# mhostetter/gr-adsb

Measured on AMD Instinct MI355X. Metric: IQ Msamples/s through framer+demod, higher is better.
Workload: dtype f32

## Files before the change

gr_adsb_amd/csrc/adsb_device.h:

```cpp
#pragma once

#ifndef ADSB_ROUTE
#define ADSB_ROUTE(id, offset) ((void)0)
#endif
#ifndef ADSB_AIR_MIN
#if defined(__HIP__)
#define ADSB_AIR_MIN(p, v) __hip_atomic_fetch_min((p), (v), __ATOMIC_RELAXED, __HIP_MEMORY_SCOPE_AGENT)
#define ADSB_AIR_LOAD(p) __hip_atomic_load((p), __ATOMIC_RELAXED, __HIP_MEMORY_SCOPE_AGENT)
#define ADSB_AIR_STORE(p, v) __hip_atomic_store((p), (v), __ATOMIC_RELAXED, __HIP_MEMORY_SCOPE_AGENT)
#else
#define ADSB_AIR_MIN(p, v) atomicMin((p), (v))
#define ADSB_AIR_LOAD(p) (*(p))
#define ADSB_AIR_STORE(p, v) ((void)(*(p) = (v)))
#endif
#endif
#ifndef ADSB_COLD_AT
#define ADSB_COLD_AT(e) (e)
#endif

namespace adsb {

enum Route : int {
  kRouteWindow = 0,
  kRoutePend = 1,
  kRoutePendFull = 2,
  kRouteFlush = 3,
  kRouteLongFast = 4,
  kRouteLongClipped = 5,
  kRouteCount = 6
};

constexpr int kThreads = 256;
constexpr int kWaves = kThreads / 64;
constexpr int kWTile = 1024;
constexpr int kFwd = 256;
constexpr int kBack = 128;
constexpr int kWWin = kWTile + kFwd;
constexpr int kMaxCentre = (kWTile - 1 + kWWin - 1) / 2;
template <bool B> struct BoolC { static constexpr bool value = B; };
constexpr int kWWords = kWWin / 64;
constexpr int kWOwn = kWTile / 64;
constexpr int kHeadWords = kFwd / 64;
constexpr unsigned kTemplate = 0x285u;
constexpr int kNoise = 100;
constexpr long long kNoIndex = -(1ll << 62);
static_assert(kWOwn == 16 && kFwd % 64 == 0, "word owners are lanes 0..15 of each wavefront");
static_assert(kBack % 64 == 0 && kBack >= 100, "the noise window of a centre in the tile must lie in the LDS window");

constexpr int kMinWaves = 5;

enum RecFlags : unsigned {
  kDemod = 1u,
  kKept = 2u,
  kNoMatch = 4u,
  kPending = 8u,
  kHead = 16u,
  kLongHint = 32u,
  kParityOk = 32u,
  kLongFmt = 64u,
  kKnownDf = 128u,
  kDfShift = 8u,
  kRecLongHint = 0x2000u,
  kFecFixed = 0x4000u,
  kFecDf = 0x8000u,
  kApFec = 4u,
  kApKnown = 8u,
};

struct CrcTab { unsigned r[112]; };
constexpr CrcTab make_crc_tab() {
  CrcTab t{};
  unsigned v = 1;
  for (int j = 0; j < 112; ++j) {
    t.r[j] = v;
    v <<= 1;
    if (v & 0x1000000u) v ^= 0x1FFF409u;
  }
  return t;
}
constexpr unsigned kDfShortSet = (1u << 0) | (1u << 4) | (1u << 5) | (1u << 11);
constexpr unsigned kDfLongSet = (1u << 16) | (1u << 17) | (1u << 18) | (1u << 19) | (1u << 20) | (1u << 21) | (1u << 24);
constexpr unsigned kDfPiSet = (1u << 11) | (1u << 17) | (1u << 18) | (1u << 19);

struct alignas(16) Rec { unsigned long long w[4]; };
struct alignas(16) RecHalf { unsigned long long a, b; };

constexpr long long kBias = 1ll << 40;
__device__ __forceinline__ unsigned long long cand_make(long long p, unsigned flags) {
  return ((unsigned long long)flags << 56) | (unsigned long long)(p + kBias);
}
__device__ __forceinline__ long long cand_p(unsigned long long c) {
  return (long long)(c & 0x00FFFFFFFFFFFFFFull) - kBias;
}
__device__ __forceinline__ unsigned cand_flags(unsigned long long c) { return (unsigned)(c >> 56); }

struct LongRise { long long rise; int blk; int slot; };

struct Summary {
  int n_rec;
  int n_kept;
  int overflow;
  int long_count;
  unsigned flags;
  int pad_;
  long long lastp;
  long long last_kept_p;
};

struct DetectArgs {
  const void* data;
  long long n;
  long long in0_base;
  long long scan_lo;
  long long scan_hi;
  long long fall_hi;
  long long dem_hi;
  long long origin;
  long long chunk;
  float thr;
  float prev_in0;
  float scale;
  int sps;
  int end_is_call_end;
  int long_aware;
  int rec_cap;
  int long_cap;
  unsigned long long* cands;
  Rec* recs;
  int* blk_count;
  long long* blk_lastp;
  unsigned* blk_flags;
  LongRise* longlist;
  int* long_count;
  unsigned long long* long_lastp;
};

__device__ __forceinline__ float mag2f(float re, float im) {
  return __fadd_rn(__fmul_rn(re, re), __fmul_rn(im, im));
}

__device__ __forceinline__ float mag2_iq16(unsigned iq, float scale) {
  const float re = __fmul_rn((float)(short)(iq & 0xFFFFu), scale);
  const float im = __fmul_rn((float)(short)(iq >> 16), scale);
  return mag2f(re, im);
}

constexpr int kModeSc8Pow2 = 5;
constexpr int kModeCu8Pow2 = 6;
template <int MODE>
__device__ __forceinline__ float mag2_iq8(unsigned iq, float scale) {
  if constexpr (MODE == 3 || MODE == kModeSc8Pow2) {
    const int i8 = (int)(signed char)(iq & 0xFFu), q8 = (int)(signed char)((iq >> 8) & 0xFFu);
    return mag2f(__fmul_rn((float)i8, scale), __fmul_rn((float)q8, scale));
  } else {
    const float fi = (float)(iq & 0xFFu), fq = (float)((iq >> 8) & 0xFFu);
    const float ci = __builtin_fmaf(fi, 2.0f, -255.0f), cq = __builtin_fmaf(fq, 2.0f, -255.0f);
    return mag2f(__fmul_rn(ci, scale), __fmul_rn(cq, scale));
  }
}

constexpr bool mode_is_iq8(int mode) { return mode == 3 || mode == 4 || mode == 5 || mode == 6; }
constexpr int det_waves(int mode) { return mode_is_iq8(mode) ? 1 : kWaves; }
constexpr int mode_bytes(int mode) { return mode == 0 ? 8 : mode_is_iq8(mode) ? 2 : 4; }

template <int MODE> struct RawSel { using type = float; };
template <> struct RawSel<0> { using type = float2; };
template <> struct RawSel<2> { using type = unsigned; };
template <> struct RawSel<3> { using type = unsigned short; };
template <> struct RawSel<4> { using type = unsigned short; };
template <> struct RawSel<5> { using type = unsigned short; };
template <> struct RawSel<6> { using type = unsigned short; };

template <int MODE>
__device__ __forceinline__ typename RawSel<MODE>::type load_raw(const void* data, long long i) {
  return reinterpret_cast<const typename RawSel<MODE>::type*>(data)[i];
}
template <int MODE>
__device__ __forceinline__ float raw_mag2(typename RawSel<MODE>::type r, float scale) {
  if constexpr (MODE == 0) return mag2f(r.x, r.y);
  else if constexpr (MODE == 2) return mag2_iq16(r, scale);
  else if constexpr (mode_is_iq8(MODE)) return mag2_iq8<MODE>(r, scale);
  else return r;
}

template <int MODE>
__device__ __forceinline__ float load_sample(const void* data, long long i, float scale) {
  return raw_mag2<MODE>(load_raw<MODE>(data, i), scale);
}

template <int MODE>
__device__ __forceinline__ float xg(const void* data, long long n, long long i, float scale) {
  if (i < 0 || i >= n) return 0.0f;
  return load_sample<MODE>(data, i, scale);
}

template <int MODE>
__device__ __forceinline__ float xg_nb(const void* data, long long n, long long i, float scale) {
  const bool ok = (i >= 0) & (i < n);
  const long long ci = ok ? i : 0;
  const float v = load_sample<MODE>(data, ci, scale);
  return ok ? v : 0.0f;
}

template <int MODE, class A>
__device__ __forceinline__ bool above_at(const A& a, long long i) {
  if (i >= 0) return xg<MODE>(a.data, a.n, i, a.scale) >= a.thr;
  if (i == a.in0_base - 1) return a.prev_in0 >= a.thr;
  return 0.0f >= a.thr;
}

__device__ __forceinline__ unsigned long long bit_range(long long lo, long long hi) {
  if (hi <= 0 || lo >= 64 || hi <= lo) return 0ull;
  if (lo < 0) lo = 0;
  if (hi > 64) hi = 64;
  unsigned long long m = (hi == 64) ? ~0ull : ((1ull << hi) - 1ull);
  return m & ~((1ull << lo) - 1ull);
}
// ... 903 lines not shown
        }
        adsb_wave_sync();

        const bool easy = it >= it_e0 && it < it_e1;
        if (easy) rises_to_records(BoolC<true>{}, it, t0, nr, lane);
        else rises_to_records(BoolC<false>{}, it, t0, nr, lane);
        adsb_setprio<0>();
      }
    }

    if (n_pend > 0 && it + 1 == ntile) {
      adsb_wave_sync();
      pend_flush<MODE, STAGED>(pend, n_pend, WinArgs<decltype(cold())>{cold(), a.origin, a.scale, a.sps}, s_x, t0, st, lane);
      n_pend = 0;
    }
    {
      const float4 keep = *reinterpret_cast<const float4*>(s_x + kWTile + 4 * lane);
      const float2 keepb = *reinterpret_cast<const float2*>(s_x + kWTile - kBack + 2 * lane);
      const unsigned short keepm = s_m16[kTileUnits + (lane & (kHeadUnits - 1))];
      adsb_wave_sync();
      *reinterpret_cast<float4*>(s_x + 4 * lane) = keep;
      *reinterpret_cast<float2*>(s_x - kBack + 2 * lane) = keepb;
      s_m16[lane & (kHeadUnits - 1)] = keepm;
    }
    pred = keepp;
    prev_active = active;
  };

  const int lane_outer = lane;
  if (cold()->n >= kWTile) {
    const char* const clamp = reinterpret_cast<const char*>(cold()->data) + (((cold()->n - kWTile) * (long long)BPS) & ~15ll);
    const char* nb = reinterpret_cast<const char*>(cold()->data) + (c0 + kFwd) * (long long)BPS;
    constexpr int D = (MODE == kModeSc8Pow2 || MODE == kModeCu8Pow2) ? 2 : 1;
    Body<MODE> body[D];
    if (ntile > 0) {
      body_issue(body[0], it_rag > 0 ? nb : clamp, lane);
#pragma unroll
      for (int d = 1; d < D; ++d) {
        nb += (long long)kWTile * BPS;
        body_issue(body[d], d - 1 < it_re ? nb : clamp, lane);
      }
      head_fill(lane);
    }
    auto step = [&](Body<MODE>& b, const int it, const bool real) {
      const int lane = adsb_opaque(lane_outer);
      const long long t0 = c0 + (long long)it * kWTile;
      nb += (long long)kWTile * BPS;
      constexpr bool MASKS = mode_is_iq8(MODE);
      unsigned bm_regs = 0u;
      bool active = false;
      const int mx = body_commit<MODE, true, MASKS>(b, s_x + kFwd, a.scale, lane, it + D - 1 < it_re ? nb : clamp, thr, thr_bits,
                                                    thr_pos, &bm_regs, &active);
      if (real) {
        if constexpr (!MASKS) active = !thr_pos || __ballot(mx >= thr_bits) != 0ull;
        if (it >= it_rag) {
          adsb_wave_sync();
          for (int i = lane; i < kWTile; i += 64) s_x[kFwd + i] = xg<MODE>(cold()->data, cold()->n, t0 + kFwd + i, a.scale);
          active = true;
        }
        process_tile(it, t0, active, lane, MASKS && it < it_rag, bm_regs);
      }
    };
    for (int it = 0; it < ntile; it += D) {
      step(body[0], it, true);
#pragma unroll
      for (int d = 1; d < D; ++d) step(body[d], it + d, it + d < ntile);
    }
  } else {
    if (ntile > 0) head_fill(lane_outer);
    for (int it = 0; it < ntile; ++it) {
      const int lane = adsb_opaque(lane_outer);
      const long long t0 = c0 + (long long)it * kWTile;
      for (int i = lane; i < kWTile; i += 64) s_x[kFwd + i] = xg<MODE>(cold()->data, cold()->n, t0 + kFwd + i, a.scale);
      process_tile(it, t0, true, lane, false, 0u);
    }
  }
  if (STAGED) stage_flush(st, nrec < a.rec_cap ? nrec : a.rec_cap, lane_outer);
#pragma unroll
  for (int d2 = 32; d2 >= 1; d2 >>= 1) lp = imax(lp, __shfl_xor(lp, d2));
  if (lane == 0) {
    cold()->blk_count[unit] = nrec;
    cold()->blk_lastp[unit] = lp >= 0 ? c0 + lp : kNoIndex;
    cold()->blk_flags[unit] = uflags;
  }
}
template <int MODE, int HALF>
__global__ void __launch_bounds__(64 * det_waves(MODE), kMinWaves) k_detect(DetectArgs a) {
  detect_body<MODE, HALF, det_waves(MODE)>(a, (int)blockIdx.x);
}

template <int MODE>
__device__ __forceinline__ void longrun_entry(const DetectArgs& a, int e) {
  __shared__ unsigned long long s_found;
  const int tid = threadIdx.x, lane = tid & 63, wave = tid >> 6;
  {
    const LongRise le = a.longlist[e];
    const long long limit = a.fall_hi;
    const long long start = le.rise + 1;
    const unsigned long long none = ~0ull;
    if (tid == 0) s_found = none;
    __syncthreads();
    for (long long base = start; base < limit; base += 4ll * kThreads) {
      unsigned long long mine = none;
      for (int q = 3; q >= 0; --q) {
        const long long i = base + 4ll * tid + q;
        if (i < limit && !above_at<MODE>(a, i)) mine = (unsigned long long)(i - start);
      }
      if (mine != none) atomicMin(&s_found, mine);
      __syncthreads();
      const bool done = s_found != none;
      __syncthreads();
      if (done) break;
    }
    __syncthreads();
    const long long f = (s_found == none) ? limit : start + (long long)s_found;
    unsigned long long* out = a.cands + (long long)le.blk * a.rec_cap + le.slot;
    if (wave == 0) {
      if (f < limit) {
        const long long p = (le.rise + f) >> 1;
        if (lane == 0) atomicMax(a.long_lastp, (unsigned long long)(p + (1ll << 62)));
        const float hp = __fmul_rn(xg<MODE>(a.data, a.n, p, a.scale), 0.5f);
        const float v = (lane < 16) ? xg<MODE>(a.data, a.n, p + (long long)lane * (a.sps >> 1), a.scale) : 0.0f;
        const unsigned long long cm = __ballot(lane < 16 && v > hp);
        unsigned hint = 0u;
        if (a.long_aware) {
          const long long i1 = p + 8ll * a.sps;
          if (xg<MODE>(a.data, a.n, i1, a.scale) > xg<MODE>(a.data, a.n, i1 + (a.sps >> 1), a.scale)) hint = kLongHint;
        }
        const bool match = (unsigned)cm == kTemplate;
        if (lane == 0) *out = match ? cand_make(p, hint) : cand_make(p, kNoMatch);
        if (match) {
          const BurstFetch<MODE> bf = burst_issue<MODE>(a, cand_make(p, hint), lane);
          burst_finish<MODE>(a, bf, a.recs + (long long)le.blk * a.rec_cap + le.slot, lane);
        }
      } else if (lane == 0) {
        *out = cand_make(le.rise, kNoMatch);
        if (!a.end_is_call_end) atomicOr(a.blk_flags + le.blk, 4u);
      }
    }
    __syncthreads();
  }
}
template <int MODE>
__device__ __forceinline__ void longrun_body(int bid, int nb, const DetectArgs& a) {
  int n_entries = *a.long_count;
  if (n_entries > a.long_cap) n_entries = a.long_cap;
  for (int e = bid; e < n_entries; e += nb) longrun_entry<MODE>(a, e);
}

__device__ __forceinline__ int block_excl_scan(int v, int* total) {
  __shared__ int s_wsum[kWaves];
  const int lane = threadIdx.x & 63, wave = threadIdx.x >> 6;
  int incl = v;
#pragma unroll
  for (int d = 1; d < 64; d <<= 1) {
    const int t = __shfl_up(incl, (unsigned)d);
    if (lane >= d) incl += t;
  }
  if (lane == 63) s_wsum[wave] = incl;
  __syncthreads();
  int base = 0, tot = 0;
#pragma unroll
  for (int w = 0; w < kWaves; ++w) {
    const int c = s_wsum[w];
    if (w < wave) base += c;
    tot += c;
// ... 2 lines not shown
  *total = tot;
  return base + incl - v;
}

constexpr int kScanRound = 512;
constexpr int kScanRoundBig = 2048;
template <int ROUND>
__device__ __forceinline__ void scan_body(const int* blk_count, const long long* blk_lastp,
                                          const unsigned* blk_flags, int nblk, int rec_cap,
                                          const int* long_count, const unsigned long long* long_lastp,
                                          int* blk_off, Summary* sum, int* s_cnt) {
  constexpr int kScanRound = ROUND;
  constexpr int kScanPer = ROUND / kThreads;
  __shared__ long long s_lp[kWaves];
  __shared__ unsigned s_fl[kWaves];
  const int tid = threadIdx.x, lane = tid & 63, wave = tid >> 6;
  long long lp = kNoIndex; unsigned fl = 0;
  int carry = 0;
  for (int base = 0; base < nblk; base += kScanRound) {
    int cc[kScanPer];
    long long ll[kScanPer];
    unsigned ff[kScanPer];
#pragma unroll
    for (int q = 0; q < kScanPer; ++q) {
      const int b = base + q * kThreads + tid, bc = b < nblk ? b : nblk - 1;
      cc[q] = blk_count[bc]; ll[q] = blk_lastp[bc]; ff[q] = blk_flags[bc];
    }
#pragma unroll
    for (int q = 0; q < kScanPer; ++q) {
      const bool in = base + q * kThreads + tid < nblk;
      int c = in ? cc[q] : 0;
      if (c > rec_cap) { fl |= 0x80000000u; c = rec_cap; }
      if (in && ll[q] > lp) lp = ll[q];
      if (in) fl |= ff[q];
      s_cnt[q * kThreads + tid] = c;
    }
    __syncthreads();
    int acc = 0;
#pragma unroll
    for (int q = 0; q < kScanPer; ++q) acc += s_cnt[tid * kScanPer + q];
    int total = 0;
    int run = carry + block_excl_scan(acc, &total);
#pragma unroll
    for (int q = 0; q < kScanPer; ++q) { const int c = s_cnt[tid * kScanPer + q]; s_cnt[tid * kScanPer + q] = run; run += c; }
    __syncthreads();
    for (int k = tid; k < kScanRound; k += kThreads)
      if (base + k < nblk) blk_off[base + k] = s_cnt[k];
    __syncthreads();
    carry += total;
  }
#pragma unroll
  for (int d = 32; d >= 1; d >>= 1) {
    const long long ol = __shfl_xor(lp, d);
    const unsigned of = __shfl_xor(fl, d);
    if (ol > lp) lp = ol;
    fl |= of;
  }
  if (lane == 0) { s_lp[wave] = lp; s_fl[wave] = fl; }
  __syncthreads();
  if (tid == 0) {
    long long L = (*long_lastp == 0ull) ? kNoIndex : (long long)(*long_lastp) - (1ll << 62);
    unsigned F = 0;
    for (int w = 0; w < kWaves; ++w) { if (s_lp[w] > L) L = s_lp[w]; F |= s_fl[w]; }
    sum->n_rec = carry; sum->overflow = (F >> 31) & 1u; sum->flags = F & 0x7FFFFFFFu; sum->lastp = L;
    sum->long_count = *long_count; sum->n_kept = 0; sum->last_kept_p = kNoIndex;
  }
}
__device__ __forceinline__ void gather_body(int bid, int nb, const unsigned long long* cands, const int* blk_count,
                                            const int* blk_off, int nblk, int rec_cap, unsigned long long* sorted,
                                            unsigned* sorted_src) {
  const int lane = threadIdx.x & 63, wave = threadIdx.x >> 6;
  for (int b = bid * kWaves + wave; b < nblk; b += nb * kWaves) {
    int c = blk_count[b];
    if (c > rec_cap) c = rec_cap;
    const int off = blk_off[b];
    const long long src = (long long)b * rec_cap;
    for (int j = lane; j < c; j += 64) {
      sorted[off + j] = cands[src + j];
      sorted_src[off + j] = (unsigned)(src + j);
    }
  }
}

constexpr int kOrderLists = kThreads;
struct OrderAcc { unsigned long long lastp_biased; unsigned flags; unsigned pad_; };
template <int MODE>
__global__ void __launch_bounds__(kThreads) k_order(DetectArgs a, int nblk, unsigned long long* sorted, unsigned* sorted_src,
                                                   Summary* sum, OrderAcc* acc) {
  __shared__ long long s_lp[kWaves];
  __shared__ unsigned s_fl[kWaves];
  const int tid = threadIdx.x, lane = tid & 63, wave = tid >> 6, bid = (int)blockIdx.x;
  const int rec_cap = a.rec_cap;
  int n_long = *a.long_count;
  if (n_long > a.long_cap) n_long = a.long_cap;
  for (int e = 0; e < n_long; ++e)
    if (a.longlist[e].blk / kOrderLists == bid) longrun_entry<MODE>(a, e);
  __syncthreads();
  const int b = bid * kOrderLists + tid;
  const bool in = b < nblk;
  const int bc = in ? b : nblk - 1;
  int cnt = a.blk_count[bc];
  long long lp = a.blk_lastp[bc];
  unsigned fl = a.blk_flags[bc];
  if (!in) { cnt = 0; lp = kNoIndex; fl = 0u; }
  if (cnt > rec_cap) { fl |= 0x80000000u; cnt = rec_cap; }
  int before = 0;
  {
    struct alignas(16) I4 { int x, y, z, w; };
    const int nfront = bid * kOrderLists;
    const I4* c4 = reinterpret_cast<const I4*>(a.blk_count);
    auto clipped = [&](const I4& v) {
      return (v.x < rec_cap ? v.x : rec_cap) + (v.y < rec_cap ? v.y : rec_cap) + (v.z < rec_cap ? v.z : rec_cap) +
             (v.w < rec_cap ? v.w : rec_cap);
    };
    const int n4 = nfront / 4;
    int i = tid;
    for (; i + 7 * kThreads < n4; i += 8 * kThreads) {
      I4 v[8];
#pragma unroll
      for (int q = 0; q < 8; ++q) v[q] = c4[i + q * kThreads];
#pragma unroll
      for (int q = 0; q < 8; ++q) before += clipped(v[q]);
    }
    for (; i < n4; i += kThreads) before += clipped(c4[i]);
  }
  int front = 0, total = 0;
  (void)block_excl_scan(before, &front);
  const int run = front + block_excl_scan(cnt, &total);
  {
    const long long src = (long long)b * rec_cap;
    constexpr int kAtOnce = 8;
    for (int j = 0; j < cnt; j += kAtOnce) {
      unsigned long long w[kAtOnce];
#pragma unroll
      for (int q = 0; q < kAtOnce; ++q) w[q] = a.cands[src + (j + q < cnt ? j + q : j)];
#pragma unroll
      for (int q = 0; q < kAtOnce; ++q)
        if (j + q < cnt) {
          sorted[run + j + q] = w[q];
          sorted_src[run + j + q] = (unsigned)(src + j + q);
        }
    }
  }
#pragma unroll
  for (int d = 32; d >= 1; d >>= 1) {
    const long long ol = __shfl_xor(lp, d);
    const unsigned of = __shfl_xor(fl, d);
    if (ol > lp) lp = ol;
    fl |= of;
  }
  if (lane == 0) { s_lp[wave] = lp; s_fl[wave] = fl; }
  __syncthreads();
  if (tid == 0) {
    long long L = kNoIndex;
    unsigned F = 0u;
    for (int w = 0; w < kWaves; ++w) { if (s_lp[w] > L) L = s_lp[w]; F |= s_fl[w]; }
    if (L != kNoIndex) atomicMax(&acc->lastp_biased, (unsigned long long)(L + (1ll << 62)));
    if (F) atomicOr(&acc->flags, F);
    if (bid == (int)gridDim.x - 1) sum->n_rec = front + total;
  }
}

__device__ __forceinline__ void resolve_body(int bid, int nb, unsigned long long* sorted, const Summary* sum, long long gate,
                                             long long gate_long, long long prev_eob) {
  const int n = sum->n_rec;
  const int nseg = (n + kThreads - 1) / kThreads;
  for (int seg = bid; seg < nseg; seg += nb) {
    const int i = seg * kThreads + threadIdx.x;
    if (i < n && !(cand_flags(sorted[i]) & kNoMatch)) {
      const long long p = cand_p(sorted[i]);
      int j = i - 1;
      while (j >= 0 && (cand_flags(sorted[j]) & kNoMatch)) --j;
      const bool head = (j < 0) || ((p - cand_p(sorted[j]) > gate_long) && (p > prev_eob));
      if (head) {
        long long eob = (j < 0) ? prev_eob : (p - 1);
        int k = i;
        while (k < n) {
          const unsigned long long ck = sorted[k];
          if (!(cand_flags(ck) & kNoMatch)) {
            const long long pk = cand_p(ck);
            if (k != i) {
              int jj = k - 1;
              while (jj >= 0 && (cand_flags(sorted[jj]) & kNoMatch)) --jj;
              if (jj >= 0 && pk - cand_p(sorted[jj]) > gate_long && pk > prev_eob) break;
            }
            if (pk > eob) {
              sorted[k] = ck | ((unsigned long long)kKept << 56);
              eob = pk + ((cand_flags(ck) & kLongHint) ? gate_long : gate);
            }
          }
          ++k;
        }
      }
    }
  }
}
__global__ void __launch_bounds__(kThreads) k_resolve(unsigned long long* sorted, const Summary* sum, long long gate,
                                                      long long gate_long, long long prev_eob) {
  resolve_body((int)blockIdx.x, (int)gridDim.x, sorted, sum, gate, gate_long, prev_eob);
}

__device__ __forceinline__ bool survives(unsigned long long c, int i, unsigned fmask, unsigned fwant, int head_n) {
  const unsigned f = cand_flags(c);
  if (f & (kNoMatch | kPending)) return false;
  return (f & fmask) == fwant || i < head_n;
}

__device__ __forceinline__ void count_body(int bid, int nb, const unsigned long long* sorted, const Summary* sum,
                                           unsigned fmask, unsigned fwant, int head_n, int* seg_count) {
  __shared__ int s_c[kWaves];
  const int n = sum->n_rec;
  const int nseg = (n + kThreads - 1) / kThreads;
  const int lane = threadIdx.x & 63, wave = threadIdx.x >> 6;
  for (int seg = bid; seg < nseg; seg += nb) {
    const int i = seg * kThreads + threadIdx.x;
    const bool kept = i < n && survives(sorted[i], i, fmask, fwant, head_n);
    const unsigned long long m = __ballot(kept);
    if (lane == 0) s_c[wave] = __popcll(m);
    __syncthreads();
    if (threadIdx.x == 0) seg_count[seg] = s_c[0] + s_c[1] + s_c[2] + s_c[3];
    __syncthreads();
  }
}
__global__ void __launch_bounds__(kThreads) k_count(const unsigned long long* sorted, const Summary* sum,
                                                    unsigned fmask, unsigned fwant, int head_n, int* seg_count) {
  count_body((int)blockIdx.x, (int)gridDim.x, sorted, sum, fmask, fwant, head_n, seg_count);
}

template <bool HOSTCOPY = false>
__device__ __forceinline__ void compact_body(int bid, int nb, const unsigned long long* sorted, const Rec* recs, const unsigned* sorted_src,
                                             Summary* sum, const int* seg_count, unsigned fmask, unsigned fwant, int head_n,
                                             Rec* out, int out_cap, int* long_count, unsigned long long* long_lastp,
                                             OrderAcc* acc = nullptr, Summary* host_sum = nullptr, Rec* host_out = nullptr,
                                             int host_cap = 0) {
  __shared__ int s_c[kWaves];
  __shared__ int s_pre[kWaves], s_tot[kWaves];
  const int n = sum->n_rec;
  const int nseg = (n + kThreads - 1) / kThreads;
  const int lane = threadIdx.x & 63, wave = threadIdx.x >> 6;
  if (bid == 0 && host_sum) {
    int tot = 0;
    for (int j = threadIdx.x; j < nseg; j += kThreads) tot += seg_count[j];
#pragma unroll
    for (int d = 32; d >= 1; d >>= 1) tot += __shfl_xor(tot, d);
    if (lane == 0) s_tot[wave] = tot;
    __syncthreads();
    tot = s_tot[0] + s_tot[1] + s_tot[2] + s_tot[3];
    __syncthreads();
    long long lastk = kNoIndex;
    if (tot > 0) {
      for (int hi = n; hi > 0 && lastk == kNoIndex; hi -= kThreads) {
        const int i = hi - 1 - (int)threadIdx.x;
        const unsigned long long c = i >= 0 ? sorted[i] : 0ull;
        const bool k = i >= 0 && survives(c, i, fmask, fwant, head_n);
        const unsigned long long m = __ballot(k);
        if (lane == 0) s_c[wave] = m ? __builtin_ctzll(m) : 64;
        __syncthreads();
        int w = 0;
        while (w < kWaves && s_c[w] == 64) ++w;
        if (w < kWaves) lastk = cand_p(sorted[hi - 1 - (w * 64 + s_c[w])]);
        __syncthreads();
      }
    }
    if (threadIdx.x == 0) {
      const unsigned F = acc->flags;
      const unsigned long long lb = acc->lastp_biased > *long_lastp ? acc->lastp_biased : *long_lastp;
      Summary f;
      f.n_rec = n; f.n_kept = tot; f.overflow = (int)((F >> 31) & 1u); f.long_count = *long_count; f.flags = F & 0x7FFFFFFFu;
      f.pad_ = 0; f.lastp = lb ? (long long)lb - (1ll << 62) : kNoIndex; f.last_kept_p = lastk;
      *host_sum = f;
      *sum = f;
      acc->flags = 0u; acc->lastp_biased = 0ull;
    }
  }
  if (bid == 0 && threadIdx.x == 0) {
    *long_count = 0;
    *long_lastp = 0ull;
    if (nseg == 0 && !host_sum) sum->n_kept = 0;
  }
  for (int seg = bid; seg < nseg; seg += nb) {
    int pre = 0, tot = 0;
    for (int j = threadIdx.x; j < nseg; j += kThreads) {
// ... 847 lines not shown
```

gr_adsb_amd/csrc/adsb_hip.hip:

```cpp
#include <hip/hip_runtime.h>

#include <pthread.h>
#include <sched.h>
#include <sys/syscall.h>
#include <unistd.h>

#include <algorithm>
#include <cerrno>
#include <cmath>
#include <cstdio>
#include <cstdlib>
#include <cstring>
#include <atomic>
#include <chrono>
#include <condition_variable>
#include <memory>
#include <mutex>
#include <new>
#include <thread>
#include <vector>

__device__ __forceinline__ void adsb_wave_sync() {
  __builtin_amdgcn_fence(__ATOMIC_RELEASE, "wavefront");
  __builtin_amdgcn_wave_barrier();
// ... 81 lines not shown
  ADSB_MAX_STEP(0x111, 0xF) ADSB_MAX_STEP(0x112, 0xF) ADSB_MAX_STEP(0x114, 0xF) ADSB_MAX_STEP(0x118, 0xF)
  ADSB_MAX_STEP(0x142, 0xA) ADSB_MAX_STEP(0x143, 0xC)
#undef ADSB_MAX_STEP
  return (unsigned)__builtin_amdgcn_readlane((int)v, 63);
}
#define ADSB_DYN_LDS_INT(name) extern __shared__ int name[]
#define ADSB_LDS __attribute__((address_space(3)))
__device__ __forceinline__ unsigned long long adsb_bitrep32(unsigned x) {
  unsigned long long r;
  asm("s_bitreplicate_b64_b32 %0, %1" : "=s"(r) : "s"(x));
  return r;
}

namespace adsb { struct DetectArgs; }
typedef const __attribute__((address_space(4))) adsb::DetectArgs* adsb_cold_ptr;
__device__ __forceinline__ adsb_cold_ptr adsb_cold(const adsb::DetectArgs&) {
  auto p = __builtin_amdgcn_kernarg_segment_ptr();
  asm volatile("" : "+s"(p));
  return (adsb_cold_ptr)p;
}
__device__ __forceinline__ adsb_cold_ptr adsb_cold_at(const adsb::DetectArgs* e) {
  unsigned long long p = (unsigned long long)e;
  asm volatile("" : "+s"(p));
  return (adsb_cold_ptr)p;
}
#define ADSB_COLD_AT(e) adsb_cold_at(e)

#include "adsb_device.h"
#include "adsb_plan.h"
#include "../../include/adsb_hip.h"

using namespace adsb;

static_assert(sizeof(adsb_burst) == 32 && sizeof(Rec) == 32, "record layout");
static_assert(sizeof(adsb_decoded) == sizeof(DecRow) && offsetof(adsb_decoded, latitude) == offsetof(DecRow, latitude) &&
              offsetof(adsb_decoded, num_msgs) == offsetof(DecRow, num_msgs), "decoded row layout");

namespace {

template <class P, auto Release>
struct Owned {
  P p = nullptr;
  Owned() = default;
  Owned(Owned&& o) noexcept : p(o.p) { o.p = nullptr; }
  ~Owned() { (void)release(); }
  hipError_t release() {
    const hipError_t e = p ? Release(p) : hipSuccess;
    p = nullptr;
    return e;
  }
  operator P() const { return p; }
  P operator->() const { return p; }
};
template <class T> using DevPtr = Owned<T*, hipFree>;
template <class T> using PinnedPtr = Owned<T*, hipHostFree>;
using Stream = Owned<hipStream_t, hipStreamDestroy>;
using Event = Owned<hipEvent_t, hipEventDestroy>;
template <auto Release>
struct Buf : Owned<void*, Release> {
  size_t cap = 0;
  hipError_t release() { cap = 0; return Owned<void*, Release>::release(); }
};
using DevBuf = Buf<hipFree>;
using PinnedBuf = Buf<hipHostFree>;

struct Misc {
  int long_count;
  int pad;
  unsigned long long long_lastp;
  OrderAcc acc;
  char fill[32];
  Summary sum;
};
static_assert(sizeof(OrderAcc) == 16, "Misc layout");

struct Slot {
  DevBuf d_cands, d_recs, d_sorted, d_sorted_src, d_out, d_seg, d_blk_count, d_blk_lastp, d_blk_flags, d_blk_off, d_long, d_misc;
  DevBuf d_in;
  DevBuf d_ratio;
  PinnedPtr<Summary> h_sum;
  PinnedBuf h_out;
  PinnedBuf h_ratio;
  Event done, ev0, ev1, det_done, h2d_done;
  Stream stream;
  hipStream_t ds = nullptr;
  hipStream_t cs = nullptr;
  bool busy = false;
  bool direct = false;
  bool fused = false;
  int host_cap = 0;
  bool is_shard = false;
  bool submitted = false;
  bool ev1_valid = false;
  bool h2d_pending = false;
  int seq = 0;
  unsigned long long air_pass = 0;
  bool air_keep = false;
  PinnedBuf h_dec;
  bool polled = false;
  Plan plan{};
  DetectArgs args{};
  int grid = 0, nlists = 0, rec_cap = 0;
  long long tot = 0, ntiles = 0, chunk = 0, span = 0;
  int32_t nres = 0;
};

struct BatchBufs {
  DevBuf d_scratch;
  DevBuf d_fixed;
  DevBuf d_da, d_ta, d_kept;
  DevBuf d_packed, d_tot;
  DevBuf d_in;
  PinnedBuf h_tab;
  PinnedBuf h_first;
  PinnedBuf h_out;
};

struct StreamState {
  long long pos = 0;
  long long eob = kStreamFreshEob;
  long long base = 0;
  long long overlong = 0;
  int cur = 0;
  int fmt = -1;
};
inline void stream_make_fresh(StreamState& s) { s.pos = 0; s.eob = kStreamFreshEob; s.overlong = 0; s.fmt = -1; }
struct StreamBufs {
  std::vector<StreamState> st;
  size_t slot_bytes = 0;
  DevBuf d_carry;
  DevBuf d_stage;
  DevBuf d_tab;
  PinnedBuf h_tab;
  PinnedBuf h_status;
};

}

struct CopyPool {
  std::vector<std::thread> th;
  std::mutex m;
  std::condition_variable cv_job, cv_done;
  const char* src = nullptr;
  char* dst = nullptr;
  size_t bytes = 0;
  unsigned gen = 0;
  int pending = 0;
  bool stop = false;
  int nthreads = 0;
  cpu_set_t cpus;
  bool have_cpus = false;

  static void slice(size_t bytes, int parts, int i, size_t* lo, size_t* hi) {
    const size_t per = ((bytes / (size_t)parts) + 4095) & ~(size_t)4095;
    *lo = per * (size_t)i < bytes ? per * (size_t)i : bytes;
    *hi = (i == parts - 1) ? bytes : (*lo + per < bytes ? *lo + per : bytes);
  }
  void worker(int id) {
    unsigned seen = 0;
    for (;;) {
      std::unique_lock<std::mutex> lk(m);
      cv_job.wait(lk, [&] { return stop || gen != seen; });
      if (stop) return;
      seen = gen;
      const char* s_ = src; char* d_ = dst; const size_t b_ = bytes;
      lk.unlock();
// ... 323 lines not shown
  hipLaunchKernelGGL(k_air_cond, dim3(1), dim3(64), 0, st, a);
  hipLaunchKernelGGL(k_air_verdict, dim3(g), dim3(kThreads), 0, st, a, 1);
  if (c->flags & ADSB_FLAG_DECODE) { int r = launch_dec(c, st, a, g, rows, ts); if (r) return r; }
  HIPCHK(c, hipEventRecord(c->air_ev, st));
  return 0;
}

int launch_air_pass(adsb_ctx* c, Slot& s, hipStream_t st, Rec* out, int force = 0) {
  AirArgs a{};
  a.out = out; a.mirror = (out != (Rec*)s.h_out.p && s.host_cap > 0) ? (Rec*)s.h_out.p : nullptr;
  a.mirror_cap = a.mirror ? s.host_cap : 0;
  a.sum = &((Misc*)s.d_misc.p)->sum; a.cap = (int)s.tot; a.host_sum = s.h_sum; a.pass = s.air_pass; a.force = force;
  if (c->flags & ADSB_FLAG_DECODE) {
    int r = ensure_pinned(c, s.h_dec, (size_t)s.tot * sizeof(DecRow));
    if (r) return r;
  }
  return launch_air(c, st, a, s.tot, (DecRow*)s.h_dec.p, nullptr);
}

int air_unbreak(adsb_ctx* c, hipStream_t st) {
  HIPCHK(c, hipStreamWaitEvent(st, c->air_ev, 0));
  HIPCHK(c, hipMemsetAsync(&c->d_air_st->broken, 0, sizeof(int), st));
  HIPCHK(c, hipEventRecord(c->air_ev, st));
  return 0;
}

int air_clear(adsb_ctx* c) {
  if (c->air_next > 0) HIPCHK(c, hipStreamWaitEvent(c->stream, c->air_ev, 0));
  HIPCHK(c, hipMemsetAsync(c->d_air, 0xFF, ((size_t)1 << 24) * sizeof(unsigned long long), c->stream));
  HIPCHK(c, hipMemsetAsync(c->d_air_st, 0, sizeof(AirState), c->stream));
  HIPCHK(c, hipEventRecord(c->air_ev, c->stream));
  c->air_next = 0;
  return 0;
}

int apply_ext(adsb_ctx* c, hipStream_t st) {
  for (int i = 0; i < c->n_ext; ++i) HIPCHK(c, hipStreamWaitEvent(st, c->ext_ev[i], 0));
  c->n_ext = 0;
  return 0;
}

int enqueue_tail(adsb_ctx* c, Slot& s) {
  const DetectArgs& a = s.args;
  const Plan& pl = s.plan;
  if (pl.air && !s.air_keep) s.air_pass = (c->air_next++) << 32;
  s.air_keep = false;
  Misc* misc = (Misc*)s.d_misc.p;
  hipStream_t ts = s.cs;
  if (s.direct) {
    ts = s.ds;
    TailArgs t;
    t.cands = a.cands; t.recs = a.recs; t.blk_count = a.blk_count; t.blk_lastp = a.blk_lastp; t.blk_flags = a.blk_flags;
    t.blk_off = (int*)s.d_blk_off.p; t.nblk = s.nlists; t.rec_cap = s.rec_cap; t.long_count = a.long_count;
    t.long_lastp = a.long_lastp; t.sorted = (unsigned long long*)s.d_sorted.p; t.sorted_src = (unsigned*)s.d_sorted_src.p;
    t.seg_count = (int*)s.d_seg.p; t.sum = &misc->sum; t.host_sum = s.h_sum; t.out = (Rec*)s.h_out.p; t.out_cap = (int)s.tot;
    t.gate_on = pl.gate ? 1 : 0; t.head_n = pl.head_n; t.gate = 63ll * c->sps;
    t.gate_long = (long long)(pl.long_aware ? 119 : 63) * c->sps; t.prev_eob = pl.prev_eob_stream - pl.origin;
    s.seq = s.seq >= 0x7FFFFFF0 ? 1 : s.seq + 1;
    t.seq = s.seq;
    if (s.fused) launch_pass_small(ts, a, t);
    else ADSB_BY_MODE(pl.mode, launch_tail_small, ts, a, t);
    if (c->flags & (ADSB_FLAG_FEC_CONSERVATIVE | ADSB_FLAG_AIRCRAFT_TABLE)) {
      if (c->flags & ADSB_FLAG_FEC_CONSERVATIVE) launch_fec(ts, s, (Rec*)s.h_out.p, &misc->sum);
      if (pl.air) { int r_ = launch_air_pass(c, s, ts, (Rec*)s.h_out.p); if (r_) return r_; }
      HIPCHK(c, hipEventRecord(s.done, ts));
      return 0;
    }
    s.polled = true;
    return 0;
  }
  if (s.ds != s.cs) {
    hipEvent_t dep = s.ev1_valid ? s.ev1 : s.det_done;
    if (!s.ev1_valid) HIPCHK(c, hipEventRecord(dep, s.ds));
    HIPCHK(c, hipStreamWaitEvent(s.cs, dep, 0));
  }
  const unsigned order_pad = (c->flags & ADSB_FLAG_LOW_LATENCY) ? 0u : 8192u;
  unsigned long long* sorted = (unsigned long long*)s.d_sorted.p;
  unsigned* sorted_src = (unsigned*)s.d_sorted_src.p;
  ADSB_BY_MODE(pl.mode, launch_order, ts, (s.nlists + kOrderLists - 1) / kOrderLists, order_pad, a, s.nlists, sorted, sorted_src,
               &misc->sum, &misc->acc);
  const int ag = 2048;
  unsigned fmask = 0u, fwant = 0u;
  if (pl.gate) {
    hipLaunchKernelGGL(k_resolve, dim3(ag), dim3(kThreads), 0, ts, sorted, (const Summary*)&misc->sum,
                       (long long)63 * c->sps, (long long)(pl.long_aware ? 119 : 63) * c->sps, pl.prev_eob_stream - pl.origin);
    fmask = kKept; fwant = kKept;
  }
  hipLaunchKernelGGL(k_count, dim3(ag), dim3(kThreads), 0, ts, (const unsigned long long*)sorted,
                     (const Summary*)&misc->sum, fmask, fwant, pl.head_n, (int*)s.d_seg.p);
  hipLaunchKernelGGL(k_compact, dim3(ag), dim3(kThreads), 0, ts, (const unsigned long long*)sorted, (const Rec*)a.recs, (const unsigned*)sorted_src,
                     &misc->sum, (const int*)s.d_seg.p, fmask, fwant, pl.head_n, (Rec*)(s.direct ? s.h_out.p : s.d_out.p), (int)s.tot,
                     a.long_count, a.long_lastp, &misc->acc, s.h_sum, (Rec*)(s.host_cap > 0 ? s.h_out.p : nullptr), s.host_cap);
  if (c->flags & ADSB_FLAG_FEC_CONSERVATIVE) launch_fec(ts, s, (Rec*)s.d_out.p, &misc->sum);
  if (pl.air) { int r_ = launch_air_pass(c, s, ts, (Rec*)s.d_out.p); if (r_) return r_; }
  HIPCHK(c, hipEventRecord(s.done, ts));
  return 0;
}

int enqueue_pass(adsb_ctx* c, Slot& s, const Plan& pl, bool submitted) {
  HIPCHK(c, hipSetDevice(c->device));
  s.plan = pl;
  s.submitted = submitted;
  s.ds = s.cs = c->stream;
  if (submitted && c->split_tail) {
    if (!c->own_stream) {
      s.cs = c->tail_stream;
    } else {
      s.ds = s.cs = s.stream;
      const long long in_bytes = (pl.scan_hi > 0 ? pl.scan_hi : 0) * (long long)mode_bytes(pl.mode);
      if ((c->flags & ADSB_FLAG_TIMING) || in_bytes > (4ll << 30) || (mode_is_iq8(pl.mode) && in_bytes >= (1ll << 30))) {
        s.ds = c->slot[0].stream;
        s.cs = c->slot[1].stream;
      }
    }
  }
  s.span = pl.scan_hi > 0 ? pl.scan_hi : 0;
  const int upb = det_waves(pl.mode);
  const int tile = kWTile;
  long long ntiles = (s.span + tile - 1) / tile;
  if (ntiles < 1) ntiles = 1;
  const int bpc = c->bpc[pl.mode];
  long long units = 0, tiles_per = 0;
  plan_chunks(ntiles, (long long)c->n_cu * bpc * upb, &units, &tiles_per);
  const long long chunk = tiles_per * tile;
  if (chunk >= (1ll << 30)) return fail(c, -EINVAL, "input too long for one call on this device (chunk per wavefront >= 2^30 samples)");
  const bool timing = (c->flags & ADSB_FLAG_TIMING) != 0;
  const bool can_fuse = units <= kWaves && pl.mode == ADSB_FMT_MAG2 && !timing;
  const int grid = can_fuse ? 1 : (int)((units + upb - 1) / upb);
  const int nlists = can_fuse ? kWaves : grid * upb;
  long long rc = (chunk / 256 + 64) << c->rec_cap_shift;
  if (rc > chunk / 2 + 8) rc = chunk / 2 + 8;
  rc = (rc + 15) & ~15ll;
  s.grid = grid; s.nlists = nlists; s.rec_cap = (int)rc; s.tot = (long long)nlists * rc; s.ntiles = ntiles; s.chunk = chunk;
  const long long long_cap = ntiles + 1;
  int r;
  if ((r = ensure(c, s.d_cands, (size_t)s.tot * 8))) return r;
  if ((r = ensure(c, s.d_recs, (size_t)s.tot * sizeof(Rec)))) return r;
  if ((r = ensure(c, s.d_sorted, (size_t)s.tot * 8))) return r;
  if (s.tot >= (1ll << 32)) return fail(c, -EINVAL, "input too long for one call (list slots >= 2^32)");
  if ((r = ensure(c, s.d_sorted_src, (size_t)s.tot * sizeof(unsigned)))) return r;
  const long long kDirectRecs = 16384;
  s.direct = s.tot <= kDirectRecs;
  const long long kMidTiles = 65536, kHostRecs = 32768;
  s.host_cap = 0;
  if (s.direct) { if ((r = ensure_pinned(c, s.h_out, (size_t)s.tot * sizeof(Rec), true))) return r; }
  else {
    if ((r = ensure(c, s.d_out, (size_t)s.tot * sizeof(Rec)))) return r;
    if (ntiles <= kMidTiles) {
      if ((r = ensure_pinned(c, s.h_out, (size_t)kHostRecs * sizeof(Rec), true))) return r;
      s.host_cap = (int)kHostRecs;
    }
  }
  if ((r = ensure(c, s.d_seg, (size_t)(s.tot / kThreads + 2) * sizeof(int)))) return r;
  if ((r = ensure(c, s.d_blk_count, (size_t)nlists * sizeof(int)))) return r;
  if ((r = ensure(c, s.d_blk_lastp, (size_t)nlists * sizeof(long long)))) return r;
  if ((r = ensure(c, s.d_blk_flags, (size_t)nlists * sizeof(unsigned)))) return r;
  if ((r = ensure(c, s.d_blk_off, (size_t)nlists * sizeof(int)))) return r;
  if ((r = ensure(c, s.d_long, (size_t)long_cap * sizeof(LongRise)))) return r;
  if (!s.d_misc.p) {
    if ((r = ensure(c, s.d_misc, sizeof(Misc)))) return r;
    HIPCHK(c, hipMemsetAsync(s.d_misc.p, 0, sizeof(Misc), s.ds));
  }
  Misc* misc = (Misc*)s.d_misc.p;

  DetectArgs& a = s.args;
  a.data = pl.d_data; a.n = pl.n; a.in0_base = pl.in0_base; a.scan_lo = pl.scan_lo; a.scan_hi = pl.scan_hi;
  a.fall_hi = pl.fall_hi; a.dem_hi = pl.dem_hi; a.origin = pl.origin; a.chunk = chunk; a.thr = c->thr;
  a.prev_in0 = pl.prev_in0; a.scale = c->scale[pl.mode]; a.sps = c->sps; a.end_is_call_end = pl.end_is_call_end; a.rec_cap = s.rec_cap;
  a.long_aware = pl.long_aware ? 1 : 0;
  a.long_cap = (int)long_cap; a.cands = (unsigned long long*)s.d_cands.p; a.recs = (Rec*)s.d_recs.p; a.blk_count = (int*)s.d_blk_count.p;
  a.blk_lastp = (long long*)s.d_blk_lastp.p; a.blk_flags = (unsigned*)s.d_blk_flags.p;
  a.longlist = (LongRise*)s.d_long.p; a.long_count = &misc->long_count; a.long_lastp = &misc->long_lastp;

  s.fused = s.direct && can_fuse;
  if (s.h2d_pending) { HIPCHK(c, hipStreamWaitEvent(s.ds, s.h2d_done, 0)); s.h2d_pending = false; }
  { int r_ = apply_ext(c, s.ds); if (r_) return r_; }
  if (!s.fused) {
    if (timing) HIPCHK(c, hipEventRecord(s.ev0, s.ds));
    ADSB_BY_MODE(pl.mode, launch_detect, c, s.ds, a, grid);
    if (timing) HIPCHK(c, hipEventRecord(s.ev1, s.ds));
  }
  c->stats.detect_grid = (uint64_t)grid; c->stats.blocks_per_cu = (uint64_t)c->bpc[pl.mode];
  c->stats.calls++;
  s.busy = true;
  s.ev1_valid = timing;
  s.polled = false;
  return enqueue_tail(c, s);
}
int enqueue(adsb_ctx* c, Slot& s, const Plan& pl, bool submitted) {
  const int r = enqueue_pass(c, s, pl, submitted);
  if (r) s.busy = false;
  return r;
}

int requeue_grown(adsb_ctx* c, Slot& s) {
  if ((long long)s.rec_cap >= s.chunk / 2 + 8) return fail(c, -EIO, "centre list overflow at maximum size");
  c->rec_cap_shift++;
  c->stats.retries++;
  const int r = enqueue(c, s, s.plan, s.submitted);
  if (r) return r;
  c->stats.calls--;
  return 0;
}

int air_settle_all(adsb_ctx* c) {
  Slot* order[ADSB_MAX_IN_FLIGHT];
  int n = 0;
  for (Slot& sl : c->slot)
    if (sl.busy && sl.plan.air) {
      int k = n++;
      for (; k > 0 && order[k - 1]->air_pass > sl.air_pass; --k) order[k] = order[k - 1];
      order[k] = &sl;
    }
  for (int i = 0; i < n; ++i) {
    Slot& s = *order[i];
    for (int attempt = 0;; ++attempt) {
      if (attempt == 16) return fail(c, -EIO, "centre list capacity did not converge");
      HIPCHK(c, hipEventSynchronize(s.done));
      HIPCHK(c, hipGetLastError());
      const hipStream_t ts = s.direct ? s.ds : s.cs;
      int r;
      if (s.h_sum->overflow) {
        if ((r = air_unbreak(c, ts))) return r;
        s.air_keep = true;
        if ((r = requeue_grown(c, s))) return r;
        continue;
      }
      if (s.h_sum->flags & kAirSkipped) {
        s.h_sum->flags &= ~kAirSkipped;
        if ((r = launch_air_pass(c, s, ts, (Rec*)(s.direct ? s.h_out.p : s.d_out.p), 1))) return r;
        HIPCHK(c, hipEventRecord(s.done, ts));
        continue;
      }
      break;
    }
  }
  return 0;
}

int finish_pass(adsb_ctx* c, Slot& s, Summary* sum, int32_t* n_res) {
  HIPCHK(c, hipSetDevice(c->device));
  const bool timing = (c->flags & ADSB_FLAG_TIMING) != 0;
  for (int attempt = 0; attempt < 16; ++attempt) {
    if (s.polled) {
      const volatile int* seqp = &s.h_sum->pad_;
      const auto t0 = std::chrono::steady_clock::now();
      unsigned spins = 0;
      while (*seqp != s.seq) {
        cpu_relax();
        if ((++spins & 0x3Fu) == 0 && std::chrono::steady_clock::now() - t0 > std::chrono::microseconds(50)) break;
      }
      std::atomic_thread_fence(std::memory_order_acquire);
      if (*seqp != s.seq) {
        HIPCHK(c, hipStreamSynchronize(s.ds));
        HIPCHK(c, hipGetLastError());
// ... 1740 lines not shown
```

Before: 776,100.

## Accumulate per-group counts in detect and fuse segment counting into gate

```diff
diff --git a/gr_adsb_amd/csrc/adsb_device.h b/gr_adsb_amd/csrc/adsb_device.h
--- a/gr_adsb_amd/csrc/adsb_device.h
+++ b/gr_adsb_amd/csrc/adsb_device.h
@@ -48,6 +48,7 @@
 static_assert(kBack % 64 == 0 && kBack >= 100, "the noise window of a centre in the tile must lie in the LDS window");
 
 constexpr int kMinWaves = 5;
+constexpr int kOrderLists = kThreads;
 
 enum RecFlags : unsigned {
   kDemod = 1u,
@@ -133,6 +134,11 @@
   LongRise* longlist;
   int* long_count;
   unsigned long long* long_lastp;
+  int* grp_count = nullptr;
+  int* grp_next = nullptr;
+  int n_grp = 0;
+  int seg_cap = 0;
+  int* seg_count = nullptr;
 };
 
 __device__ __forceinline__ float mag2f(float re, float im) {
@@ -1202,6 +1208,8 @@
     cold()->blk_count[unit] = nrec;
     cold()->blk_lastp[unit] = lp >= 0 ? c0 + lp : kNoIndex;
     cold()->blk_flags[unit] = uflags;
+    int* const grp = cold()->grp_count;
+    if (grp) atomicAdd(grp + unit / kOrderLists, nrec < a.rec_cap ? nrec : a.rec_cap);
   }
 }
 template <int MODE, int HALF>
@@ -1370,7 +1378,6 @@
   }
 }
 
-constexpr int kOrderLists = kThreads;
 struct OrderAcc { unsigned long long lastp_biased; unsigned flags; unsigned pad_; };
 template <int MODE>
 __global__ void __launch_bounds__(kThreads) k_order(DetectArgs a, int nblk, unsigned long long* sorted, unsigned* sorted_src,
@@ -1392,8 +1399,17 @@
   unsigned fl = a.blk_flags[bc];
   if (!in) { cnt = 0; lp = kNoIndex; fl = 0u; }
   if (cnt > rec_cap) { fl |= 0x80000000u; cnt = rec_cap; }
+  if (a.seg_count) {
+    const int per = (a.seg_cap + (int)gridDim.x - 1) / (int)gridDim.x;
+    const int lo = bid * per, hi = lo + per < a.seg_cap ? lo + per : a.seg_cap;
+    for (int j = lo + tid; j < hi; j += kThreads) a.seg_count[j] = 0;
+  }
+  if (bid == 0 && a.grp_next)
+    for (int j = tid; j < a.n_grp; j += kThreads) a.grp_next[j] = 0;
   int before = 0;
-  {
+  if (a.grp_count) {
+    for (int g = tid; g < bid; g += kThreads) before += a.grp_count[g];
+  } else {
     struct alignas(16) I4 { int x, y, z, w; };
     const int nfront = bid * kOrderLists;
     const I4* c4 = reinterpret_cast<const I4*>(a.blk_count);
@@ -1449,13 +1465,16 @@
   }
 }
 
+template <bool COUNT = false>
 __device__ __forceinline__ void resolve_body(int bid, int nb, unsigned long long* sorted, const Summary* sum, long long gate,
-                                             long long gate_long, long long prev_eob) {
+                                             long long gate_long, long long prev_eob, int head_n = 0, int* seg_count = nullptr) {
   const int n = sum->n_rec;
   const int nseg = (n + kThreads - 1) / kThreads;
   for (int seg = bid; seg < nseg; seg += nb) {
     const int i = seg * kThreads + threadIdx.x;
+    int mine = 0;
     if (i < n && !(cand_flags(sorted[i]) & kNoMatch)) {
+      if (COUNT && i < head_n && !(cand_flags(sorted[i]) & kPending)) mine = 1;
       const long long p = cand_p(sorted[i]);
       int j = i - 1;
       while (j >= 0 && (cand_flags(sorted[j]) & kNoMatch)) --j;
@@ -1463,6 +1482,7 @@
       if (head) {
         long long eob = (j < 0) ? prev_eob : (p - 1);
         int k = i;
+        int far_seg = seg, far = 0;
         while (k < n) {
           const unsigned long long ck = sorted[k];
           if (!(cand_flags(ck) & kNoMatch)) {
@@ -1475,17 +1495,38 @@
             if (pk > eob) {
               sorted[k] = ck | ((unsigned long long)kKept << 56);
               eob = pk + ((cand_flags(ck) & kLongHint) ? gate_long : gate);
+              if (COUNT && k >= head_n && !(cand_flags(ck) & kPending)) {
+                const int ks = k / kThreads;
+                if (ks == seg) ++mine;
+                else {
+                  if (ks != far_seg) {
+                    if (far) atomicAdd(seg_count + far_seg, far);
+                    far_seg = ks; far = 0;
+                  }
+                  ++far;
+                }
+              }
             }
           }
           ++k;
         }
+        if (COUNT && far) atomicAdd(seg_count + far_seg, far);
       }
+    }
+    if (COUNT) {
+#pragma unroll
+      for (int d = 32; d >= 1; d >>= 1) mine += __shfl_xor(mine, d);
+      if ((threadIdx.x & 63) == 0 && mine) atomicAdd(seg_count + seg, mine);
     }
   }
 }
 __global__ void __launch_bounds__(kThreads) k_resolve(unsigned long long* sorted, const Summary* sum, long long gate,
                                                       long long gate_long, long long prev_eob) {
   resolve_body((int)blockIdx.x, (int)gridDim.x, sorted, sum, gate, gate_long, prev_eob);
+}
+__global__ void __launch_bounds__(kThreads) k_gate(unsigned long long* sorted, const Summary* sum, long long gate, long long gate_long,
+                                                   long long prev_eob, int head_n, int* seg_count) {
+  resolve_body<true>((int)blockIdx.x, (int)gridDim.x, sorted, sum, gate, gate_long, prev_eob, head_n, seg_count);
 }
 
 __device__ __forceinline__ bool survives(unsigned long long c, int i, unsigned fmask, unsigned fwant, int head_n) {
diff --git a/gr_adsb_amd/csrc/adsb_hip.hip b/gr_adsb_amd/csrc/adsb_hip.hip
--- a/gr_adsb_amd/csrc/adsb_hip.hip
+++ b/gr_adsb_amd/csrc/adsb_hip.hip
@@ -187,6 +187,8 @@
   PinnedBuf h_out;
   PinnedBuf h_ratio;
   Event done, ev0, ev1, det_done, h2d_done;
+  DevBuf d_grp;
+  int grp_half = 0, grp_cur = 0;
   Stream stream;
   hipStream_t ds = nullptr;
   hipStream_t cs = nullptr;
@@ -676,12 +678,14 @@
   const int ag = 2048;
   unsigned fmask = 0u, fwant = 0u;
   if (pl.gate) {
-    hipLaunchKernelGGL(k_resolve, dim3(ag), dim3(kThreads), 0, ts, sorted, (const Summary*)&misc->sum,
-                       (long long)63 * c->sps, (long long)(pl.long_aware ? 119 : 63) * c->sps, pl.prev_eob_stream - pl.origin);
+    hipLaunchKernelGGL(k_gate, dim3(ag), dim3(kThreads), 0, ts, sorted, (const Summary*)&misc->sum,
+                       (long long)63 * c->sps, (long long)(pl.long_aware ? 119 : 63) * c->sps, pl.prev_eob_stream - pl.origin,
+                       pl.head_n, (int*)s.d_seg.p);
     fmask = kKept; fwant = kKept;
-  }
-  hipLaunchKernelGGL(k_count, dim3(ag), dim3(kThreads), 0, ts, (const unsigned long long*)sorted,
-                     (const Summary*)&misc->sum, fmask, fwant, pl.head_n, (int*)s.d_seg.p);
+  } else {
+    hipLaunchKernelGGL(k_count, dim3(ag), dim3(kThreads), 0, ts, (const unsigned long long*)sorted,
+                       (const Summary*)&misc->sum, fmask, fwant, pl.head_n, (int*)s.d_seg.p);
+  }
   hipLaunchKernelGGL(k_compact, dim3(ag), dim3(kThreads), 0, ts, (const unsigned long long*)sorted, (const Rec*)a.recs, (const unsigned*)sorted_src,
                      &misc->sum, (const int*)s.d_seg.p, fmask, fwant, pl.head_n, (Rec*)(s.direct ? s.h_out.p : s.d_out.p), (int)s.tot,
                      a.long_count, a.long_lastp, &misc->acc, s.h_sum, (Rec*)(s.host_cap > 0 ? s.h_out.p : nullptr), s.host_cap);
@@ -745,7 +749,8 @@
       s.host_cap = (int)kHostRecs;
     }
   }
-  if ((r = ensure(c, s.d_seg, (size_t)(s.tot / kThreads + 2) * sizeof(int)))) return r;
+  const long long seg_cap = s.tot / kThreads + 2;
+  if ((r = ensure(c, s.d_seg, (size_t)seg_cap * sizeof(int)))) return r;
   if ((r = ensure(c, s.d_blk_count, (size_t)nlists * sizeof(int)))) return r;
   if ((r = ensure(c, s.d_blk_lastp, (size_t)nlists * sizeof(long long)))) return r;
   if ((r = ensure(c, s.d_blk_flags, (size_t)nlists * sizeof(unsigned)))) return r;
@@ -756,6 +761,16 @@
     HIPCHK(c, hipMemsetAsync(s.d_misc.p, 0, sizeof(Misc), s.ds));
   }
   Misc* misc = (Misc*)s.d_misc.p;
+  const int ngrp = (nlists + kOrderLists - 1) / kOrderLists;
+  if (!s.direct) {
+    if (ngrp > s.grp_half) {
+      if ((r = ensure(c, s.d_grp, (size_t)2 * ngrp * sizeof(int)))) return r;
+      s.grp_half = (int)(s.d_grp.cap / (2 * sizeof(int)));
+      s.grp_cur = 0;
+      HIPCHK(c, hipMemsetAsync(s.d_grp.p, 0, s.d_grp.cap, s.ds));
+    }
+    s.grp_cur ^= 1;
+  }
 
   DetectArgs& a = s.args;
   a.data = pl.d_data; a.n = pl.n; a.in0_base = pl.in0_base; a.scan_lo = pl.scan_lo; a.scan_hi = pl.scan_hi;
@@ -765,6 +780,13 @@
   a.long_cap = (int)long_cap; a.cands = (unsigned long long*)s.d_cands.p; a.recs = (Rec*)s.d_recs.p; a.blk_count = (int*)s.d_blk_count.p;
   a.blk_lastp = (long long*)s.d_blk_lastp.p; a.blk_flags = (unsigned*)s.d_blk_flags.p;
   a.longlist = (LongRise*)s.d_long.p; a.long_count = &misc->long_count; a.long_lastp = &misc->long_lastp;
+  a.grp_count = a.grp_next = a.seg_count = nullptr; a.n_grp = a.seg_cap = 0;
+  if (!s.direct) {
+    a.grp_count = (int*)s.d_grp.p + (size_t)s.grp_cur * s.grp_half;
+    a.grp_next = (int*)s.d_grp.p + (size_t)(s.grp_cur ^ 1) * s.grp_half;
+    a.n_grp = s.grp_half;
+    if (pl.gate) { a.seg_count = (int*)s.d_seg.p; a.seg_cap = (int)seg_cap; }
+  }
 
   s.fused = s.direct && can_fuse;
   if (s.h2d_pending) { HIPCHK(c, hipStreamWaitEvent(s.ds, s.h2d_done, 0)); s.h2d_pending = false; }
```

After: 730,100. 0.941x the previous value.
